# godk1122/IsaacLab

Measured on AMD Instinct MI355X. Metric: env-steps/sec (whole node), Anymal-C rough 4096 envs/GPU, RSL-RL PPO iteration (collect+GAE+update), higher is better.
Workload: dtype f32; 1 GPU; Isaac-Velocity-Rough-Anymal-C-v0, 4096 envs/GPU, T=24, 5 epochs x 4 minibatches, terrain 1204008 triangles, 4 state snapshots resident in HBM; parallelism=dp1, rollout=hipGraph, full_step=False, update=hipGraph (measured eager 16.00 ms, graph 15.55 ms), policy_params=571801

## Files before the change

include/imx.h:

```cpp
#ifndef IMX_H_
#define IMX_H_

#include <stddef.h>
#include <stdint.h>

#ifdef __cplusplus
extern "C" {
#endif

typedef struct imx_plan imx_plan_t;
typedef struct imx_mesh imx_mesh_t;
typedef void* imx_stream_t;

#define IMX_MAGIC 0x31584D49
#define IMX_PLAN_VERSION 3
#define IMX_HEADER_WORDS 48
#define IMX_MAX_OBS_GROUPS 4
#define IMX_REC_WORDS 20
#define IMX_FRAME_WORDS 9
#define IMX_FT_HEADER_WORDS 4

enum imx_header_word {
    IMX_H_MAGIC = 0, IMX_H_VERSION, IMX_H_J, IMX_H_B, IMX_H_H, IMX_H_A, IMX_H_D, IMX_H_R, IMX_H_NTERM, IMX_H_NREW,
    IMX_H_NOBS, IMX_H_NACT, IMX_H_MAX_EP_LEN, IMX_H_STEP_DT , IMX_H_TERM_OFF, IMX_H_REW_OFF, IMX_H_OBS_OFF,
// ... 408 lines not shown
size_t imx_gae_scratch_bytes(int64_t T, int64_t N);
int imx_gae(int64_t T, int64_t N, const float* rewards_d, const float* values_d, const uint8_t* dones_d,
            const float* last_values_d, float gamma, float lam, int normalize, float* returns_d,
            float* advantages_d, void* scratch_d, imx_stream_t stream);

size_t imx_ppo_scratch_bytes(int64_t M);
int imx_ppo_loss_fwd(int64_t M, int64_t A, const float* mu_d, const float* sigma_d, int64_t sigma_stride,
                     const float* actions_d, const float* old_logp_d, const float* old_mu_d, const float* old_sigma_d,
                     const float* advantages_d, const float* returns_d, const float* values_d, const float* old_values_d,
                     float clip_param, int use_clipped_value_loss, float value_loss_coef, float entropy_coef,
                     float* out8_d, float* accum5_d, void* scratch_d, imx_stream_t stream);
int imx_ppo_loss_bwd(int64_t M, int64_t A, const float* mu_d, const float* sigma_d, int64_t sigma_stride,
                     const float* actions_d, const float* old_logp_d, const float* advantages_d, const float* returns_d,
                     const float* values_d, const float* old_values_d, float clip_param, int use_clipped_value_loss,
                     float value_loss_coef, float entropy_coef, float grad_scale, float* dmu_d, float* dsigma_d,
                     float* dvalue_d, imx_stream_t stream);

size_t imx_colsum_scratch_bytes(void);
int imx_colsum(int64_t M, int64_t A, const float* x_d, const float* y_d, float* out_d, void* scratch_d, imx_stream_t stream);

int imx_adam_step(int64_t n, float* param_d, const float* grad_d, float* exp_avg_d, float* exp_avg_sq_d,
                  const float* lr_d, const float* grad_norm_d, float max_norm, float beta1, float beta2, float eps,
                  int64_t step, imx_stream_t stream);

int imx_adam_update(int64_t n, float* param_d, const float* grad_d, float* exp_avg_d, float* exp_avg_sq_d, float* state8_d,
                    const float* kl_d, float desired_kl, const float* grad_norm_d, float max_norm, float beta1,
                    float beta2, float eps, imx_stream_t stream);

size_t imx_adam_norm_scratch_bytes(int64_t n);
int imx_adam_update_norm(int64_t n, float* param_d, const float* grad_d, float* exp_avg_d, float* exp_avg_sq_d, float* state8_d,
                         const float* kl_d, float desired_kl, float max_norm, float beta1, float beta2, float eps,
                         void* scratch_d, size_t scratch_bytes, imx_stream_t stream);

int imx_gather_rows(int64_t M, const int64_t* idx_d, int n, const void* const* src_d, void* const* dst_d,
                    const int32_t* width_floats, imx_stream_t stream);
int imx_gather_rows_pitched(int64_t M, const int64_t* idx_d, int n, const void* const* src_d, void* const* dst_d,
                            const int32_t* width_floats, const int32_t* dst_pitch_floats, imx_stream_t stream);

int imx_policy_act(int64_t N, int64_t A, int64_t D, const float* mu_d, const float* std_d, const float* value_d,
                   const float* obs_d, uint64_t seed, const int32_t* step_counter_d, float* actions_out_d,
                   float* logp_out_d, float* mu_out_d, float* sigma_out_d, float* values_out_d, float* obs_out_d,
                   float* actions_env_d, imx_stream_t stream);

int imx_rollout_post(int64_t N, const float* reward_d, const uint8_t* terminated_d, const uint8_t* truncated_d,
                     const float* value_t_d, float gamma, int bootstrap_time_outs, float* rewards_out_d,
                     uint8_t* dones_out_d, int64_t* dones_long_d, float* cur_reward_sum_d, float* cur_ep_len_d,
                     float* ep_stats3_d, const float* log_in_d, float* log_accum_d, int num_log, imx_stream_t stream);


int imx_contact_sensor_update(int64_t N, int64_t B, int64_t H, const float* new_net_forces_d, float dt, float update_period,
                              float force_threshold, int track_air_time, float* timestamp_d,
                              float* timestamp_last_update_d, uint8_t* is_outdated_d, float* net_forces_w_d,
                              float* net_forces_w_history_d, float* last_air_time_d, float* current_air_time_d,
                              float* last_contact_time_d, float* current_contact_time_d, imx_stream_t stream);

int imx_velocity_command(int64_t N, const float* cfg15, int heading_command, float dt, int do_compute,
                         const float* root_quat_w_d,
                         const float* root_lin_vel_w_d, const float* root_ang_vel_w_d, const uint8_t* reset_mask_d,
                         const float* uniforms_d, uint64_t seed, const int32_t* step_counter_d, float* vel_command_b_d,
                         float* heading_target_d, uint8_t* is_heading_env_d, uint8_t* is_standing_env_d,
                         float* time_left_d, int64_t* command_counter_d, float* metric_error_vel_xy_d,
                         float* metric_error_vel_yaw_d, imx_stream_t stream);

int imx_pose_command(int64_t N, const float* cfg16, int make_quat_unique, int64_t body_idx, int64_t num_bodies, float dt,
                     int do_compute, const float* root_pos_w_d, const float* root_quat_w_d, const float* body_pos_w_d,
                     const float* body_quat_w_d, const uint8_t* reset_mask_d, const float* uniforms_d, uint64_t seed,
// ... 22 lines not shown
                          const float* weights_d, int64_t num_weights, const float* joint_pos_target_d, const float* joint_pos_d,
                          const float* joint_vel_d, float* hidden_state_d, float* cell_state_d, float saturation_effort,
                          const float* effort_limit_d, const float* velocity_limit_d, float* computed_effort_d,
                          float* applied_effort_d, imx_stream_t stream);

int imx_actuator_net_mlp(int64_t N, int64_t J, int num_dense, const int32_t* dense_out_h, int act, const float* weights_d,
                         int64_t num_weights, int history_length, const int32_t* input_idx_d, int num_idx, float pos_scale,
                         float vel_scale, float torque_scale, int vel_first, const float* joint_pos_target_d,
                         const float* joint_pos_d, const float* joint_vel_d, float* pos_error_history_d, float* vel_history_d,
                         float saturation_effort, const float* effort_limit_d, const float* velocity_limit_d,
                         float* computed_effort_d, float* applied_effort_d, imx_stream_t stream);

int imx_empirical_normalization(int64_t N, int64_t D, const float* x_d, int update, float eps, float* mean_d, float* var_d,
                                float* std_d, int64_t* count_d, float* out_d, imx_stream_t stream);

typedef struct imx_norm_group imx_norm_group_t;
typedef struct imx_infer_norm imx_infer_norm_t;
#include "imx_normalization_struct.h"
size_t imx_empirical_normalization_partials_bytes(int64_t N, int64_t D);
int imx_empirical_normalization_update(int ngroups, const imx_norm_group_t* groups, imx_stream_t stream);


size_t imx_mlp_scratch_bytes(int64_t M, int out_features, int in_features);

int imx_mlp_dw(int64_t M, int N, int K, const float* dY_d, int64_t ldy, const float* X_d, int64_t ldx, float* dW_d,
               float* db_d, void* scratch_d, size_t scratch_bytes, imx_stream_t stream);

typedef struct imx_reduce_batch imx_reduce_batch_t;
int imx_reduce_batch_create(imx_reduce_batch_t** out);
void imx_reduce_batch_destroy(imx_reduce_batch_t* batch);
int imx_mlp_set_dw_cu_budget(int cus);
int imx_reduce_batch_begin(imx_reduce_batch_t* batch);
int imx_reduce_batch_flush(imx_reduce_batch_t* batch, imx_stream_t stream);

int imx_mlp_dw_elu(int64_t M, int N, int K, const float* dH_d, int64_t ldg, const float* H_d, int64_t ldh, float elu_alpha,
                   float* dZ_out_d, int64_t ldd, const float* X_d, int64_t ldx, float* dW_d, float* db_d, void* scratch_d,
                   size_t scratch_bytes, imx_stream_t stream);

int imx_mlp_infer(int64_t M, const float* X_d, int64_t ldx, int nnets, const int* nlayers, const int* dims,
                  const float* const* weights_d, const int* weight_pitch, const float* const* biases_d, const float* elu_alpha,
                  float* const* out_d, imx_stream_t stream);

typedef struct imx_policy_act {
    const float* std_d;
    uint64_t seed;
    const int32_t* step_counter_d;
    float* actions_out_d;
    float* logp_out_d;
    float* mu_out_d;
    float* sigma_out_d;
    float* obs_out_d;
    const imx_plan_t* plan;
    const imx_state_t* state;
    const imx_buffers_t* buf;
    float pre_clip;
} imx_policy_act_t;
int imx_mlp_infer_act(int64_t M, const float* X_d, int64_t ldx, int nnets, const int* nlayers, const int* dims,
                      const float* const* weights_d, const int* weight_pitch, const float* const* packed_weights_d,
                      const float* const* biases_d, const float* elu_alpha, float* const* out_d, const imx_policy_act_t* act,
                      imx_stream_t stream);
int imx_mlp_infer_act2(int64_t M, const float* const* X_d, const int64_t* ldx, int nnets, const int* nlayers, const int* dims,
                       const float* const* weights_d, const int* weight_pitch, const float* const* packed_weights_d,
                       const float* const* biases_d, const float* elu_alpha, float* const* out_d, const imx_policy_act_t* act,
                       float* critic_obs_out_d, imx_stream_t stream);
int imx_mlp_infer_act2n(int64_t M, const float* const* X_d, const int64_t* ldx, int nnets, const int* nlayers, const int* dims,
                        const float* const* weights_d, const int* weight_pitch, const float* const* packed_weights_d,
// ... 112 lines not shown
```

isaaclab_amd/csrc/mlp.hip:

```cpp
#include <algorithm>

#include "imx_internal.h"
#include "imx_infer_device.h"


namespace {

constexpr int DW_T = 128;
constexpr int DW_BM = 32;
constexpr int DW_LD = DW_T + 32;

struct DwArgs {
    int64_t M;
    int N, K;
    const float* dY;
    int64_t ldy;
    const float* X;
    int64_t ldx;
    float* part;
    float* part_db;
    int tn, tk, S;
    int64_t rps;
    const float* H;
    int64_t ldh;
// ... 929 lines not shown
        else if (xvec) IMX_DW_LAUNCH(false, true, true);
        else IMX_DW_LAUNCH(false, false, true);
    } else {
        if (yvec && xvec) IMX_DW_LAUNCH(true, true, false);
        else if (yvec) IMX_DW_LAUNCH(true, false, false);
        else if (xvec) IMX_DW_LAUNCH(false, true, false);
        else IMX_DW_LAUNCH(false, false, false);
    }
#undef IMX_DW_LAUNCH
    IMX_HIP(hipGetLastError());
    return reduce_or_defer(who, (int64_t)N * K, p.S, a.part, dW_d, N, a.part_db, db_d, st);
}

extern "C" int imx_reduce_batch_create(imx_reduce_batch_t** out) {
    IMX_REQUIRE(out, "imx_reduce_batch_create: null argument");
    *out = new imx_reduce_batch();
    (*out)->args.n = 0;
    (*out)->blocks = 0;
    return 0;
}

extern "C" void imx_reduce_batch_destroy(imx_reduce_batch_t* b) {
    if (t_batch == b) t_batch = nullptr;
    delete b;
}

extern "C" int imx_reduce_batch_begin(imx_reduce_batch_t* b) {
    IMX_REQUIRE(b, "imx_reduce_batch_begin: null batch");
    IMX_REQUIRE(t_batch == nullptr, "imx_reduce_batch_begin: another batch is still open on this thread (flush it first)");
    t_batch = b;
    return 0;
}

extern "C" int imx_reduce_batch_flush(imx_reduce_batch_t* b, imx_stream_t stream) {
    IMX_REQUIRE(b && t_batch == b, "imx_reduce_batch_flush: this batch is not the one open on this thread");
    t_batch = nullptr;
    if (b->args.n == 0) return 0;
    hipLaunchKernelGGL(k_mlp_reduce_batch, dim3(b->blocks), dim3(64, RED_Y), 0, (hipStream_t)stream, b->args);
    b->args.n = 0;
    b->blocks = 0;
    IMX_HIP(hipGetLastError());
    return 0;
}

extern "C" int imx_mlp_dw(int64_t M, int N, int K, const float* dY_d, int64_t ldy, const float* X_d, int64_t ldx, float* dW_d,
                          float* db_d, void* scratch_d, size_t scratch_bytes, imx_stream_t stream) {
    return mlp_dw_launch("imx_mlp_dw", M, N, K, dY_d, ldy, nullptr, 0, 0.0f, nullptr, 0, X_d, ldx, dW_d, db_d, scratch_d, scratch_bytes,
                         stream);
}

extern "C" int imx_mlp_dw_elu(int64_t M, int N, int K, const float* dH_d, int64_t ldg, const float* H_d, int64_t ldh, float elu_alpha,
                              float* dZ_out_d, int64_t ldd, const float* X_d, int64_t ldx, float* dW_d, float* db_d, void* scratch_d,
                              size_t scratch_bytes, imx_stream_t stream) {
    IMX_REQUIRE(H_d, "imx_mlp_dw_elu: the saved activation output is required");
    return mlp_dw_launch("imx_mlp_dw_elu", M, N, K, dH_d, ldg, H_d, ldh, elu_alpha, dZ_out_d, ldd, X_d, ldx, dW_d, db_d, scratch_d,
                         scratch_bytes, stream);
}

static int head_fwd_launch(int64_t M, int K, int A, float* h_d, int64_t ldh, const float* W_d, const float* b_d, float* y_d,
                           int elu_in_place, float elu_alpha, const imx_head_loss_t* loss, imx_stream_t stream) {
    IMX_REQUIRE(M > 0 && h_d && W_d && b_d && y_d, "imx_mlp_head_fwd: bad arguments");
    IMX_REQUIRE(A >= 1 && A <= HEAD_A, "imx_mlp_head_fwd: %d outputs (1..%d supported; wider layers are library GEMMs)", A, HEAD_A);
    IMX_REQUIRE(K >= 16 && K % 16 == 0 && K <= 2048 && ldh >= K && ldh % 4 == 0 && aligned16(h_d),
                "imx_mlp_head_fwd: in-features %d (pitch %lld) must be a multiple of 16, 16-byte aligned rows", K, (long long)ldh);
    IMX_REQUIRE((size_t)A * K * sizeof(float) <= 64 * 1024, "imx_mlp_head_fwd: %d x %d weights do not fit the 64 KB of LDS used", A, K);
    imx_head_loss_t L{};
    int mode = 0;
    if (loss) {
        L = *loss;
        mode = L.mode;
        IMX_REQUIRE(mode == 1 || mode == 2, "imx_mlp_head_fwd_loss: mode %d (1 policy, 2 value)", mode);
        if (mode == 1) {
            IMX_REQUIRE(L.sigma_d && L.actions_d && L.old_logp_d && L.advantages_d && L.dmu_d && L.dsigma_d, "imx_mlp_head_fwd_loss: null policy argument");
            IMX_REQUIRE(L.sigma_stride == 0 || L.sigma_stride == A, "imx_mlp_head_fwd_loss: sigma_stride must be 0 (shared std) or A");
        } else {
// ... 519 lines not shown
```

isaaclab_amd/csrc/rollout.hip:

```cpp
#include "imx_internal.h"

struct Mom {
    float n, mean, m2;
};
IMX_DEV Mom mom_merge(Mom a, Mom b) {
    Mom r;
    r.n = a.n + b.n;
    if (r.n == 0.0f) { r.mean = 0.0f; r.m2 = 0.0f; return r; }
    const float d = b.mean - a.mean;
    r.mean = a.mean + d * (b.n / r.n);
    r.m2 = a.m2 + b.m2 + d * d * (a.n * b.n / r.n);
    return r;
}
IMX_DEV Mom mom_wave(Mom m) {
#pragma unroll
    for (int o = 32; o > 0; o >>= 1) {
        Mom b;
        b.n = __shfl_xor(m.n, o, 64);
        b.mean = __shfl_xor(m.mean, o, 64);
        b.m2 = __shfl_xor(m.m2, o, 64);
        const bool lo = ((threadIdx.x & o) == 0);
        m = lo ? mom_merge(m, b) : mom_merge(b, m);
    }
    return m;
// ... 456 lines not shown
}

extern "C" int imx_adam_update(int64_t n, float* p, const float* g, float* m, float* v, float* state8, const float* kl_d,
                               float desired_kl, const float* grad_norm_d, float max_norm, float beta1, float beta2,
                               float eps, imx_stream_t stream) {
    IMX_REQUIRE(n > 0 && p && g && m && v && state8, "imx_adam_update: bad arguments");
    hipLaunchKernelGGL(k_adam_prepare, dim3(1), dim3(64), 0, (hipStream_t)stream, state8, kl_d, desired_kl, grad_norm_d,
                       max_norm, beta1, beta2);
    const unsigned grid = (unsigned)std::min<int64_t>((n + 255) / 256, 2048);
    hipLaunchKernelGGL(k_adam_apply, dim3(grid), dim3(256), 0, (hipStream_t)stream, n, p, g, m, v, (const float*)state8, beta1,
                       beta2, eps);
    IMX_HIP(hipGetLastError());
    return 0;
}


static int adam_norm_blocks(int64_t n) {
    return (int)((n + (int64_t)ADAM_NORM_BLOCK * ADAM_NORM_PER_THREAD - 1) / ((int64_t)ADAM_NORM_BLOCK * ADAM_NORM_PER_THREAD));
}

extern "C" size_t imx_adam_norm_scratch_bytes(int64_t n) { return n > 0 ? ((size_t)adam_norm_blocks(n) + 1) * sizeof(float) : 0; }

extern "C" int imx_adam_update_norm(int64_t n, float* p, const float* g, float* m, float* v, float* state8, const float* kl_d,
                                    float desired_kl, float max_norm, float beta1, float beta2, float eps, void* scratch_d,
                                    size_t scratch_bytes, imx_stream_t stream) {
    IMX_REQUIRE(n > 0 && p && g && m && v && state8 && scratch_d, "imx_adam_update_norm: bad arguments");
    const int G = adam_norm_blocks(n);
    IMX_REQUIRE(scratch_bytes >= ((size_t)G + 1) * sizeof(float), "imx_adam_update_norm: scratch too small (see imx_adam_norm_scratch_bytes)");
    hipLaunchKernelGGL(k_adam_norm_prepare, dim3((unsigned)G), dim3(ADAM_NORM_BLOCK), 0, (hipStream_t)stream, n, g, state8, kl_d, desired_kl,
                       max_norm, beta1, beta2, (float*)scratch_d);
    const unsigned grid = (unsigned)std::min<int64_t>((n + 255) / 256, 2048);
    hipLaunchKernelGGL(k_adam_apply, dim3(grid), dim3(256), 0, (hipStream_t)stream, n, p, g, m, v, (const float*)state8, beta1,
                       beta2, eps);
    IMX_HIP(hipGetLastError());
    return 0;
}

struct GatherArgs {
    const float* src[12];
    float* dst[12];
    int width[12];
    int dpitch[12];
    int offset[13];
    int n;
};
__global__ void __launch_bounds__(256) k_gather_rows(int64_t M, const int64_t* __restrict__ idx, GatherArgs a) {
    const int lane = threadIdx.x & 63;
    const int64_t wave = ((int64_t)blockIdx.x * blockDim.x + threadIdx.x) >> 6, nw = ((int64_t)gridDim.x * blockDim.x) >> 6;
    for (int64_t r0 = 2 * wave; r0 < M; r0 += 2 * nw) {
        const int64_t r1 = r0 + 1;
        const bool two = r1 < M;
        const int64_t s0 = idx[r0], s1 = two ? idx[r1] : 0;
        for (int k = 0; k < a.n; ++k) {
            const int w = a.width[k], dp = a.dpitch[k];
            const float* __restrict__ src = a.src[k];
            float* __restrict__ dst = a.dst[k];
            for (int c = lane; c < w; c += 64) {
                const float v0 = src[s0 * w + c];
                const float v1 = two ? src[s1 * w + c] : 0.0f;
                dst[r0 * dp + c] = v0;
                if (two) dst[r1 * dp + c] = v1;
            }
        }
    }
}

// ... 158 lines not shown
```

isaaclab_amd/rsl_rl/ppo.py:

```python

from __future__ import annotations

import ctypes
import os

import torch
import torch.distributed as dist
import torch.nn as nn
import torch.nn.functional as F

from .. import _lib
from .._lib import check, lib
from .storage import RolloutStorage


class _FusedPPOLoss(torch.autograd.Function):
    @staticmethod
    def forward(ctx, mu, sigma, value, actions, old_logp, old_mu, old_sigma, adv, ret, old_value, clip, clipped, vcoef, ecoef):
        L = lib()
        M, A = mu.shape
        mu_c, sg_c, v_c = mu.contiguous(), sigma.contiguous(), value.contiguous()
        args = [t.contiguous() for t in (actions, old_logp, old_mu, old_sigma, adv, ret, old_value)]
        actions, old_logp, old_mu, old_sigma, adv, ret, old_value = args
        out8 = torch.empty(8, device=mu.device)
        scratch = torch.empty(int(L.imx_ppo_scratch_bytes(M)), dtype=torch.uint8, device=mu.device)
        check(L.imx_ppo_loss_fwd(M, A, mu_c.data_ptr(), sg_c.data_ptr(), A, actions.data_ptr(), old_logp.data_ptr(),
                                 old_mu.data_ptr(), old_sigma.data_ptr(), adv.data_ptr(), ret.data_ptr(), v_c.data_ptr(),
                                 old_value.data_ptr(), float(clip), int(clipped), float(vcoef), float(ecoef),
                                 out8.data_ptr(), None, scratch.data_ptr(), _lib.current_stream(mu.device)))
        ctx.save_for_backward(mu_c, sg_c, v_c, actions, old_logp, adv, ret, old_value)
        ctx.cfg = (float(clip), int(clipped), float(vcoef), float(ecoef))
        stats = out8[:4]
        ctx.mark_non_differentiable(stats)
        return out8[4], stats

    @staticmethod
    def backward(ctx, g_loss, _g_stats):
        mu, sigma, value, actions, old_logp, adv, ret, old_value = ctx.saved_tensors
        clip, clipped, vcoef, ecoef = ctx.cfg
        M, A = mu.shape
        dmu, dsigma, dvalue = torch.empty_like(mu), torch.empty_like(sigma), torch.empty_like(value)
        check(lib().imx_ppo_loss_bwd(M, A, mu.data_ptr(), sigma.data_ptr(), A, actions.data_ptr(), old_logp.data_ptr(),
                                     adv.data_ptr(), ret.data_ptr(), value.data_ptr(), old_value.data_ptr(), clip, clipped,
                                     vcoef, ecoef, 1.0, dmu.data_ptr(), dsigma.data_ptr(), dvalue.data_ptr(),
# ... 178 lines not shown

FUSED_L0 = os.getenv("IMX_FUSED_L0", "1") != "0"
FUSED_HEAD = os.getenv("IMX_FUSED_HEAD", "0")
LOSS_ON_SIDE = os.getenv("IMX_LOSS_ON_SIDE", "1") == "1"


def fused_first_layer_ok(x: torch.Tensor, w: torch.Tensor) -> bool:
    return (x.is_cuda and x.dtype == torch.float32 and x.stride(1) == 1 and w.is_contiguous() and w.shape[1] == x.shape[1]
            and x.shape[1] <= FUSED_FIRST_LAYER_MAX_K and FUSED_L0)


def mlp_scratch(layers, M: int, device) -> torch.Tensor:
    n = max(int(lib().imx_mlp_scratch_bytes(M, lin.out_features, lin.in_features)) for lin, _ in layers)
    return torch.empty(n, dtype=torch.uint8, device=device)


class DeferredReductions:

    def __init__(self, layers, M: int, device):
        import ctypes

        L = lib()
        self.scratch = [torch.empty(int(L.imx_mlp_scratch_bytes(M, lin.out_features, lin.in_features)), dtype=torch.uint8, device=device)
                        for lin, _ in layers]
        h = ctypes.c_void_p()
        check(L.imx_reduce_batch_create(ctypes.byref(h)))
        self.handle = h

    def __del__(self):
        try:
            lib().imx_reduce_batch_destroy(self.handle)
        except Exception:
            pass


def _head_bwd_args(scratch, which="a"):
    mode = FUSED_HEAD
    if mode == "0" or (mode == "c" and which != "c") or (mode == "a" and which != "a"):
        return None
    if isinstance(scratch, DeferredReductions):
        return {"scratch": scratch.scratch[-1], "batch": scratch.handle}
    return {"scratch": scratch, "batch": None}


def mlp_forward(layers, x, out=None, head_loss=None, first=None):
    saved = [x]
    h = x
    pending_elu = None
    for li, (lin, act) in enumerate(layers):
        if li == 0 and first is not None:
            h = first
            saved.append(h)
            continue
        if act is None and _is_head(lin, h):
            if out is not None and li == len(layers) - 1:
                z = out
            else:
                z = torch.empty(h.shape[0], lin.out_features, device=h.device, dtype=h.dtype)
            fb = head_loss.get("bwd") if head_loss is not None and li == len(layers) - 1 else None
            if (fb is not None and lin.in_features in (128, 256) and lin.out_features <= 16 and h.stride(0) % 4 == 0
                    and (pending_elu is not None or li == 0 or layers[li - 1][1] is None)):
                scr = fb["scratch"]
                dprev = torch.empty(h.shape[0], lin.in_features, device=h.device, dtype=h.dtype)
                check(lib().imx_mlp_head_fwd_bwd(h.shape[0], lin.in_features, lin.out_features, h.data_ptr(), h.stride(0), lin.weight.data_ptr(),
                                                 lin.bias.data_ptr(), z.data_ptr(), int(pending_elu is not None), float(pending_elu or 0.0),
                                                 ctypes.byref(head_loss["loss"]), dprev.data_ptr(), lin.weight.grad.data_ptr(),
# ... 15 lines not shown
        else:
            if pending_elu is not None:
                h = F.elu(h, alpha=pending_elu, inplace=True)
                pending_elu = None
            if li == 0 and isinstance(act, nn.ELU) and li + 1 < len(layers) - 1 and fused_first_layer_ok(h, lin.weight):
                z = torch.empty(h.shape[0], lin.out_features, device=h.device)
                check(lib().imx_mlp_fwd_elu(h.shape[0], lin.out_features, lin.in_features, h.data_ptr(), h.stride(0), lin.weight.data_ptr(),
                                            lin.bias.data_ptr(), float(act.alpha), 1, z.data_ptr(), z.stride(0), _lib.current_stream(h.device)))
                h = z
                saved.append(h)
                continue
            z = torch.addmm(lin.bias, h, lin.weight.t())
        if act is None:
            h = z
        elif isinstance(act, nn.ELU):
            nxt = layers[li + 1][0] if li + 1 < len(layers) else None
            if nxt is not None and layers[li + 1][1] is None and _is_head(nxt, z) and li + 1 == len(layers) - 1:
                pending_elu = float(act.alpha)
                h = z
            else:
                h = F.elu(z, alpha=act.alpha, inplace=True)
            saved.append(h)
        else:
            h = act(z)
            saved.append((z, h))
    if pending_elu is not None:
        h = F.elu(h, alpha=pending_elu, inplace=True)
    if out is not None and h is not out:
        out.copy_(h)
        h = out
    return h, saved


def mlp_backward(layers, saved, dout, scratch=None, head_dprev=None):
    L = lib()
    M = dout.shape[0]
    if scratch is None:
        scratch = mlp_scratch(layers, M, dout.device)
    stream = _lib.current_stream(dout.device)
    deferred = scratch if isinstance(scratch, DeferredReductions) else None
    if deferred is not None:
        check(L.imx_reduce_batch_begin(deferred.handle))
    try:
        _mlp_backward_layers(L, layers, saved, dout, M, scratch, deferred, stream, head_dprev)
    finally:
        if deferred is not None:
            check(L.imx_reduce_batch_flush(deferred.handle, stream))


def _mlp_backward_layers(L, layers, saved, dout, M, scratch, deferred, stream, head_dprev=None):
    d = dout
    pending = None
    top = len(layers) - 1
    if head_dprev is not None:
        d, top = head_dprev, top - 1
    for i in range(top, -1, -1):
        lin, _ = layers[i]
        x = saved[i] if not isinstance(saved[i], tuple) else saved[i][1]
        prev_act = layers[i - 1][1] if i > 0 else None
        N, K = lin.out_features, lin.in_features
        scr = deferred.scratch[i] if deferred is not None else scratch
        if pending is not None:
            dh, h, alpha = pending
            pending = None
            d = torch.empty_like(dh) if i > 0 else None
            check(L.imx_mlp_dw_elu(M, N, K, dh.data_ptr(), dh.stride(0), h.data_ptr(), h.stride(0), float(alpha),
                                   _lib.ptr(d), N, x.data_ptr(), x.stride(0), lin.weight.grad.data_ptr(),
                                   lin.bias.grad.data_ptr(), scr.data_ptr(), scr.numel(), stream))
        else:
            if not d.is_contiguous():
                d = d.contiguous()
            if i > 0 and _is_head(lin, x) and (prev_act is None or isinstance(prev_act, nn.ELU)):
                dprev = torch.empty(M, K, device=d.device, dtype=d.dtype)
                check(L.imx_mlp_head_bwd(M, K, N, d.data_ptr(), x.data_ptr(), x.stride(0), lin.weight.data_ptr(),
                                         float(prev_act.alpha) if prev_act is not None else 0.0, int(prev_act is not None),
                                         dprev.data_ptr(), lin.weight.grad.data_ptr(), lin.bias.grad.data_ptr(),
                                         scr.data_ptr(), scr.numel(), stream))
                d = dprev
                continue
            check(L.imx_mlp_dw(M, N, K, d.data_ptr(), d.stride(0), x.data_ptr(), x.stride(0), lin.weight.grad.data_ptr(),
                               lin.bias.grad.data_ptr(), scr.data_ptr(), scr.numel(), stream))
        if i > 0:
            dx = torch.mm(d, lin.weight)
            if isinstance(prev_act, nn.ELU) and dx.stride(1) == 1 and saved[i].stride(1) == 1:
                pending = (dx, saved[i], prev_act.alpha)
            elif isinstance(prev_act, nn.ELU):
                d = torch.ops.aten.elu_backward(dx, prev_act.alpha, 1.0, 1.0, True, saved[i])
            elif prev_act is None:
                d = dx
            else:
                z, h = saved[i]
                d = _act_backward(prev_act, dx, z, h)


def _act_backward(act, dh, z, h):
    if isinstance(act, nn.Identity):
        return dh
    if isinstance(act, nn.Tanh):
        return torch.ops.aten.tanh_backward(dh, h)
    if isinstance(act, nn.Sigmoid):
        return torch.ops.aten.sigmoid_backward(dh, h)
    if isinstance(act, nn.ReLU):
        return torch.ops.aten.threshold_backward(dh, h, 0)
    if isinstance(act, nn.LeakyReLU):
        return torch.ops.aten.leaky_relu_backward(dh, z, act.negative_slope, False)
    if isinstance(act, nn.SELU):
        return torch.ops.aten.elu_backward(dh, 1.6732632423543772848170429916717, 1.0507009873554804934193349852946, 1.0, False, z)
    with torch.inference_mode(False), torch.enable_grad():
        zz = z.clone().requires_grad_(True)
        (d,) = torch.autograd.grad(act(zz), zz, dh.clone())
    return d


class PPO:
# ... 5 lines not shown
        if kwargs:
            raise NotImplementedError("PPO got arguments it does not implement: " + ", ".join(sorted(kwargs)))
        if rnd_cfg is not None or symmetry_cfg is not None:
            raise NotImplementedError("RND / symmetry augmentation are outside the hot-path scope (SURVEY.md section 8)")
        self.device = torch.device(device)
        self.is_multi_gpu = multi_gpu_cfg is not None
        if self.is_multi_gpu:
            self.gpu_global_rank = multi_gpu_cfg["global_rank"]
            self.gpu_world_size = multi_gpu_cfg["world_size"]
        else:
            self.gpu_global_rank, self.gpu_world_size = 0, 1
        self.policy = policy.to(self.device)
        pair = self._first_layer_pair()
        self.bucket = FlatParams(self.policy, extra_slots=8,
                                 first=() if pair is None else (pair[0].weight, pair[1].weight, pair[0].bias, pair[1].bias))
        self._joint0 = None
        if pair is not None:
            la, lc, _alpha = pair
            H, K = la.out_features, la.in_features
            if (lc.weight.data_ptr() == la.weight.data_ptr() + 4 * H * K and lc.bias.data_ptr() == la.bias.data_ptr() + 4 * H
                    and la.weight.is_contiguous() and lc.weight.is_contiguous()):
                w0 = self.bucket.flat[:2 * H * K].view(2 * H, K)
                b0 = self.bucket.flat[2 * H * K:2 * H * K + 2 * H]
                if w0.data_ptr() == la.weight.data_ptr() and b0.data_ptr() == la.bias.data_ptr():
                    self._joint0 = (w0, b0, H, float(pair[2]))
        self.storage: RolloutStorage | None = None
        self.transition = RolloutStorage.Transition()
        self.clip_param, self.num_learning_epochs, self.num_mini_batches = clip_param, num_learning_epochs, num_mini_batches
        self.value_loss_coef, self.entropy_coef, self.gamma, self.lam = value_loss_coef, entropy_coef, gamma, lam
        self.max_grad_norm, self.use_clipped_value_loss = max_grad_norm, use_clipped_value_loss
        self.desired_kl, self.schedule = desired_kl, schedule
        self.normalize_advantage_per_mini_batch = normalize_advantage_per_mini_batch
        self.betas, self.eps = (0.9, 0.999), 1e-8
        self._adam = torch.tensor([float(learning_rate), 0.0, 1.0, 1.0, 1.0, 0.0, 1.0, 0.0], device=self.device)
        self._stats = torch.zeros(5, device=self.device)
        self._out8 = self.bucket.grad[self.bucket.numel:self.bucket.numel + 8]
        self._kl = self._out8[3:4]
        self._norm_scratch = torch.zeros(int(lib().imx_adam_norm_scratch_bytes(self.bucket.numel)), dtype=torch.uint8, device=self.device) \
            if self.device.type == "cuda" else None
        self._actor_layers = _mlp_layers(self.policy.actor)
        self._critic_layers = _mlp_layers(self.policy.critic)
        self._ws: dict = {}
        self._side = None
        if self.device.type == "cuda" and os.getenv("IMX_DW_CU_BUDGET"):
            lib().imx_mlp_set_dw_cu_budget(int(os.environ["IMX_DW_CU_BUDGET"]))
        self.two_streams = bool(two_streams)
        if self.device.type == "cuda":
            for st in (self._side_stream(), self._aux_stream()):
                if st is not None:
                    with torch.cuda.stream(st):
                        torch.zeros(1, device=self.device)
            torch.cuda.synchronize(self.device)

    @property
    def learning_rate(self) -> float:
        return float(self._adam[0].item())

    def optimizer_state_dict(self) -> dict:
        base = self.bucket.flat.data_ptr()
        state, params = {}, []
        step = self._adam[1:2].clone().reshape(())
        for i, p in enumerate(q for q in self.policy.parameters() if q.requires_grad):
            off = (p.data_ptr() - base) // 4
            params.append(i)
            if float(step) > 0:
                state[i] = {"step": step.clone(), "exp_avg": self.bucket.exp_avg[off:off + p.numel()].view_as(p).clone(),
                            "exp_avg_sq": self.bucket.exp_avg_sq[off:off + p.numel()].view_as(p).clone()}
# ... 100 lines not shown
    time_allreduce = False
    _allreduce_events: list = []

    def reduce_parameters(self):
        if self.time_allreduce and self.device.type == "cuda":
            e0, e1 = torch.cuda.Event(enable_timing=True), torch.cuda.Event(enable_timing=True)
            e0.record()
            allreduce_mean_(self.bucket.grad, self.gpu_world_size)
            e1.record()
            self._allreduce_events.append((e0, e1))
            return
        allreduce_mean_(self.bucket.grad, self.gpu_world_size)

    def allreduce_us(self) -> dict | None:
        ev, self._allreduce_events = self._allreduce_events, []
        if not ev:
            return None
        ev[-1][1].synchronize()
        t = [a.elapsed_time(b) * 1e3 for a, b in ev]
        return {"mean": sum(t) / len(t), "max": max(t), "count": len(t)}

    def _side_stream(self):
        if not self.two_streams or self.device.type != "cuda":
            return None
        if self._side is None:
            self._side = torch.cuda.Stream(self.device)
        return self._side

    def _aux_stream(self):
        if getattr(self, "_aux", None) is None:
            self._aux = torch.cuda.Stream(self.device)
        return self._aux

    def _workspace(self, M: int, A: int):
        ws = self._ws.get((M, A))
        if ws is None:
            dev = self.device
            ws = dict(dmu=torch.empty(M, A, device=dev), dsigma=torch.empty(M, A, device=dev), dvalue=torch.empty(M, 1, device=dev),
                      scratch=torch.empty(int(lib().imx_ppo_scratch_bytes(M)), dtype=torch.uint8, device=dev),
                      colsum=torch.empty(int(lib().imx_colsum_scratch_bytes()), dtype=torch.uint8, device=dev),
                      mlp_a=DeferredReductions(self._actor_layers, M, dev), mlp_c=DeferredReductions(self._critic_layers, M, dev))
            self._ws[(M, A)] = ws
        return ws

    def minibatch_step(self, obs, critic_obs, actions, target_values, advantages, returns, old_logp, old_mu, old_sigma):
        L = lib()
        pol = self.policy
        stream = _lib.current_stream(self.device)
        M, A = actions.shape
        for name, t in (("actions", actions), ("target_values", target_values), ("advantages", advantages), ("returns", returns),
                        ("old_actions_log_prob", old_logp), ("old_mu", old_mu), ("old_sigma", old_sigma)):
            if not t.is_contiguous():
                raise _lib.ImxError(f"PPO.minibatch_step: {name} must be contiguous (shape {tuple(t.shape)}, strides {t.stride()})")
        ws = self._workspace(M, A)
        if pol.noise_std_type == "scalar":
            sigma, sstride = pol.std, 0
        else:
            sigma, sstride = None, A
        clipf, vclip = float(self.clip_param), int(self.use_clipped_value_loss)
        vcoef, ecoef = float(self.value_loss_coef), float(self.entropy_coef)

        heads = {"a": None, "c": None}

        def actor_pass(st):
            nonlocal sigma
            hl = None
# ... 24 lines not shown
            if not hl.get("applied"):
                check(L.imx_ppo_loss_bwd(M, A, None, None, sstride, None, None, None, returns.data_ptr(), value.data_ptr(),
                                         target_values.data_ptr(), clipf, vclip, vcoef, ecoef, 1.0, None, None, ws["dvalue"].data_ptr(), st))
            return value, saved_c

        def loss_values(mu, value, st):
            check(L.imx_ppo_loss_fwd(M, A, mu.data_ptr(), sigma.data_ptr(), sstride, actions.data_ptr(), old_logp.data_ptr(),
                                     old_mu.data_ptr(), old_sigma.data_ptr(), advantages.data_ptr(), returns.data_ptr(),
                                     value.data_ptr(), target_values.data_ptr(), clipf, vclip, vcoef, ecoef,
                                     self._out8.data_ptr(), self._stats.data_ptr(), ws["scratch"].data_ptr(), st))
            if pol.noise_std_type == "scalar" and A <= 64:
                check(L.imx_colsum(M, A, ws["dsigma"].data_ptr(), None, pol.std.grad.data_ptr(), ws["colsum"].data_ptr(), st))
            elif A <= 64:
                check(L.imx_colsum(M, A, ws["dsigma"].data_ptr(), sigma.data_ptr(), pol.log_std.grad.data_ptr(), ws["colsum"].data_ptr(), st))
            elif pol.noise_std_type == "scalar":
                torch.sum(ws["dsigma"], dim=0, out=pol.std.grad)
            else:
                torch.sum(ws["dsigma"] * sigma, dim=0, out=pol.log_std.grad)

        first_a = first_c = z0 = None
        joint_elu = None
        if self._joint0 is not None and critic_obs.data_ptr() == obs.data_ptr() and critic_obs.shape == obs.shape:
            w0, b0, H0, alpha0 = self._joint0
            if fused_first_layer_ok(obs, w0):
                z0 = torch.empty(obs.shape[0], 2 * H0, device=obs.device)
                check(L.imx_mlp_fwd_elu(obs.shape[0], 2 * H0, obs.shape[1], obs.data_ptr(), obs.stride(0), w0.data_ptr(), b0.data_ptr(),
                                        alpha0, 1, z0.data_ptr(), z0.stride(0), stream))
            else:
                z0 = torch.addmm(b0, obs, w0.t())
                joint_elu = alpha0
            first_a, first_c = z0[:, :H0], z0[:, H0:]
        side = self._side_stream()
        main = torch.cuda.current_stream(self.device)
        if side is not None:
            loss_on_side = LOSS_ON_SIDE
            aux = self._aux_stream()
            side.wait_stream(main)
            if joint_elu is not None:
                F.elu(first_a, alpha=joint_elu, inplace=True)
            mu, saved_a = actor_pass(stream)
            mu_ready = torch.cuda.Event()
            mu_ready.record(main)
            with torch.cuda.stream(side):
                if joint_elu is not None:
                    F.elu(first_c, alpha=joint_elu, inplace=True)
                value, saved_c = critic_pass(side.cuda_stream)
                value_ready = torch.cuda.Event()
                value_ready.record(side)
            if not loss_on_side:
                aux.wait_stream(main)
                aux.wait_event(value_ready)
            mlp_backward(self._actor_layers, saved_a, ws["dmu"], ws["mlp_a"], head_dprev=heads["a"])
            with torch.cuda.stream(side):
                mlp_backward(self._critic_layers, saved_c, ws["dvalue"], ws["mlp_c"], head_dprev=heads["c"])
                if loss_on_side:
                    side.wait_event(mu_ready)
                    loss_values(mu, value, side.cuda_stream)
            if not loss_on_side:
                with torch.cuda.stream(aux):
                    loss_values(mu, value, aux.cuda_stream)
            main.wait_stream(side)
            if not loss_on_side:
                main.wait_stream(aux)
            mu.record_stream(aux)
            mu.record_stream(side)
            value.record_stream(aux)
            value.record_stream(main)
            if z0 is not None:
                z0.record_stream(side)
        else:
            if joint_elu is not None:
                F.elu(z0, alpha=joint_elu, inplace=True)
            mu, saved_a = actor_pass(stream)
            value, saved_c = critic_pass(stream)
            loss_values(mu, value, stream)
            mlp_backward(self._actor_layers, saved_a, ws["dmu"], ws["mlp_a"], head_dprev=heads["a"])
            mlp_backward(self._critic_layers, saved_c, ws["dvalue"], ws["mlp_c"], head_dprev=heads["c"])
        return self._out8

    update_graph = False
    _update_calls = 0
    _update_g = None
    _update_t = None

    @torch.no_grad()
    def update(self):
        if not (self.update_graph and self.device.type == "cuda" and not self.is_multi_gpu) or self._update_t == "eager":
            return self._update_eager()
        self._update_calls += 1
        c = self._update_calls
        if c == 1:
            return self._update_eager()
        if c == 2:
            ev = [torch.cuda.Event(enable_timing=True) for _ in range(4)]
            self._update_ev = ev
            ev[0].record()
            out = self._update_eager()
            ev[1].record()
            return out
        if c == 5 and self._update_t is None and os.getenv("IMX_UPDATE_GRAPH") == "force":
            self._update_t = "graph"
        if c == 5 and self._update_t is None:
            ev = self._update_ev
            ev[3].synchronize()
            t_eager, t_graph = ev[0].elapsed_time(ev[1]), ev[2].elapsed_time(ev[3])
            self._update_times_ms = (t_eager, t_graph)
            self._update_t = "graph" if t_graph < t_eager else "eager"
            if self._update_t == "eager":
                self._update_g = None
                return self._update_eager()
# ... 7 lines not shown
            if c == 4:
                self._update_ev[2].record()
            self._update_g.replay()
            if c == 4:
                self._update_ev[3].record()
        self.storage.clear()
        return self._stats

    def _update_eager(self):
        b = self.bucket
        L = lib()
        stream = _lib.current_stream(self.device)
        self._stats.zero_()
        adaptive = self.desired_kl is not None and self.schedule == "adaptive"
        side = self._side_stream()
        copy_stream = self._aux_stream() if side is not None else None
        main = torch.cuda.current_stream(self.device) if side is not None else None
        gen = iter(self.storage.mini_batch_generator(self.num_mini_batches, self.num_learning_epochs, copy_stream=copy_stream))
        item = next(gen, None)
        while item is not None:
            if copy_stream is not None:
                batch, ready = item
                main.wait_event(ready)
            else:
                batch = item
            if self.normalize_advantage_per_mini_batch:
                batch = list(batch)
                adv = batch[4]
                batch[4] = (adv - adv.mean()) / (adv.std() + 1e-8)
            self.minibatch_step(*batch)
            item = next(gen, None)
            if self.is_multi_gpu:
                self.reduce_parameters()
            check(L.imx_adam_update_norm(b.numel, b.flat.data_ptr(), b.grad.data_ptr(), b.exp_avg.data_ptr(), b.exp_avg_sq.data_ptr(),
                                         self._adam.data_ptr(), self._kl.data_ptr() if adaptive else None,
                                         float(self.desired_kl or 0.0), float(self.max_grad_norm or 0.0), self.betas[0],
                                         self.betas[1], self.eps, self._norm_scratch.data_ptr(), self._norm_scratch.numel(), stream))
        if copy_stream is not None:
            main.wait_stream(copy_stream)
        self.storage.clear()
        return self._stats

    def loss_dict(self) -> dict:
        s = self._stats.tolist()
        n = max(s[4], 1.0)
        return {"value_function": s[0] / n, "surrogate": s[1] / n, "entropy": s[2] / n, "kl": s[3] / n}
```

Baseline: 5.484 million env-steps/s.

## Compute Adam grad-norm partials early during backward and split update kernel

Splits the fused Adam norm+update into a block-partial squared-norm kernel and an apply kernel. The partial sums for actor parameter blocks above the input layer are computed during the backward pass, once their gradients are final, so only the remaining late blocks are reduced before the update. The Adam state is double-banked so the apply kernel can read the old state and write a new one without a separate finalize kernel. This shortens the serial tail after backward, but adds launches, a 4096-thread-block tree reduction, and host-side bank bookkeeping that must stay consistent with graph capture.

Result: no change. 5.481 million env-steps/s (-0.0%).

```diff
diff --git a/include/imx.h b/include/imx.h
--- a/include/imx.h
+++ b/include/imx.h
@@ -464,6 +464,13 @@
                          const float* kl_d, float desired_kl, float max_norm, float beta1, float beta2, float eps,
                          void* scratch_d, size_t scratch_bytes, imx_stream_t stream);
 
+#define IMX_ADAM_NORM_BLOCK 4096
+int imx_adam_norm_partials(int64_t n, const float* grad_d, const int32_t* blocks_d, int count, void* scratch_d, size_t scratch_bytes,
+                           imx_stream_t stream);
+int imx_adam_update_partials(int64_t n, float* param_d, const float* grad_d, float* exp_avg_d, float* exp_avg_sq_d,
+                             const float* state8_in_d, float* state8_out_d, const float* kl_d, float desired_kl, float max_norm,
+                             float beta1, float beta2, float eps, const void* scratch_d, size_t scratch_bytes, imx_stream_t stream);
+
 int imx_gather_rows(int64_t M, const int64_t* idx_d, int n, const void* const* src_d, void* const* dst_d,
                     const int32_t* width_floats, imx_stream_t stream);
 int imx_gather_rows_pitched(int64_t M, const int64_t* idx_d, int n, const void* const* src_d, void* const* dst_d,
@@ -552,6 +559,7 @@
 int imx_mlp_set_dw_cu_budget(int cus);
 int imx_reduce_batch_begin(imx_reduce_batch_t* batch);
 int imx_reduce_batch_flush(imx_reduce_batch_t* batch, imx_stream_t stream);
+int imx_reduce_batch_flush_queued(imx_reduce_batch_t* batch, imx_stream_t stream);
 
 int imx_mlp_dw_elu(int64_t M, int N, int K, const float* dH_d, int64_t ldg, const float* H_d, int64_t ldh, float elu_alpha,
                    float* dZ_out_d, int64_t ldd, const float* X_d, int64_t ldx, float* dW_d, float* db_d, void* scratch_d,
diff --git a/isaaclab_amd/csrc/mlp.hip b/isaaclab_amd/csrc/mlp.hip
--- a/isaaclab_amd/csrc/mlp.hip
+++ b/isaaclab_amd/csrc/mlp.hip
@@ -985,15 +985,24 @@
     return 0;
 }
 
-extern "C" int imx_reduce_batch_flush(imx_reduce_batch_t* b, imx_stream_t stream) {
-    IMX_REQUIRE(b && t_batch == b, "imx_reduce_batch_flush: this batch is not the one open on this thread");
-    t_batch = nullptr;
+static int reduce_batch_launch(imx_reduce_batch* b, imx_stream_t stream) {
     if (b->args.n == 0) return 0;
     hipLaunchKernelGGL(k_mlp_reduce_batch, dim3(b->blocks), dim3(64, RED_Y), 0, (hipStream_t)stream, b->args);
     b->args.n = 0;
     b->blocks = 0;
     IMX_HIP(hipGetLastError());
     return 0;
+}
+
+extern "C" int imx_reduce_batch_flush(imx_reduce_batch_t* b, imx_stream_t stream) {
+    IMX_REQUIRE(b && t_batch == b, "imx_reduce_batch_flush: this batch is not the one open on this thread");
+    t_batch = nullptr;
+    return reduce_batch_launch(b, stream);
+}
+
+extern "C" int imx_reduce_batch_flush_queued(imx_reduce_batch_t* b, imx_stream_t stream) {
+    IMX_REQUIRE(b && t_batch == b, "imx_reduce_batch_flush_queued: this batch is not the one open on this thread");
+    return reduce_batch_launch(b, stream);
 }
 
 extern "C" int imx_mlp_dw(int64_t M, int N, int K, const float* dY_d, int64_t ldy, const float* X_d, int64_t ldx, float* dW_d,
diff --git a/isaaclab_amd/csrc/rollout.hip b/isaaclab_amd/csrc/rollout.hip
--- a/isaaclab_amd/csrc/rollout.hip
+++ b/isaaclab_amd/csrc/rollout.hip
@@ -512,6 +512,104 @@
     const unsigned grid = (unsigned)std::min<int64_t>((n + 255) / 256, 2048);
     hipLaunchKernelGGL(k_adam_apply, dim3(grid), dim3(256), 0, (hipStream_t)stream, n, p, g, m, v, (const float*)state8, beta1,
                        beta2, eps);
+    IMX_HIP(hipGetLastError());
+    return 0;
+}
+
+static_assert(ADAM_NORM_BLOCK * ADAM_NORM_PER_THREAD == IMX_ADAM_NORM_BLOCK, "imx.h: IMX_ADAM_NORM_BLOCK");
+
+IMX_DEV float adam_norm_tree(float* red, float s) {
+    red[threadIdx.x] = s;
+    __syncthreads();
+    for (int w = ADAM_NORM_BLOCK / 2; w > 0; w >>= 1) {
+        if ((int)threadIdx.x < w) red[threadIdx.x] += red[threadIdx.x + w];
+        __syncthreads();
+    }
+    return red[0];
+}
+
+__global__ void __launch_bounds__(ADAM_NORM_BLOCK)
+k_adam_norm_partials(int64_t n, const float* __restrict__ g, const int32_t* __restrict__ blocks, int G, float* __restrict__ scratch) {
+    __shared__ float red[ADAM_NORM_BLOCK];
+    const int b = blocks[blockIdx.x];
+    if (b < 0 || b >= G) return;
+    const int64_t base = (int64_t)b * ADAM_NORM_BLOCK * ADAM_NORM_PER_THREAD;
+    float s = 0.0f;
+#pragma unroll
+    for (int k = 0; k < ADAM_NORM_PER_THREAD; ++k) {
+        const int64_t i = base + (int64_t)k * ADAM_NORM_BLOCK + threadIdx.x;
+        if (i < n) s += g[i] * g[i];
+    }
+    const float tot = adam_norm_tree(red, s);
+    if (threadIdx.x == 0) scratch[b] = tot;
+}
+
+__global__ void __launch_bounds__(ADAM_NORM_BLOCK)
+k_adam_apply_partials(int64_t n, float* __restrict__ p, const float* __restrict__ g, float* __restrict__ m, float* __restrict__ v,
+                      const float* __restrict__ st, float* __restrict__ st_out, const float* __restrict__ kl_d, float desired_kl,
+                      float max_norm, float b1, float b2, float eps, const float* __restrict__ scratch, int G) {
+    __shared__ float red[ADAM_NORM_BLOCK];
+    const int64_t stride = (int64_t)gridDim.x * blockDim.x;
+    int64_t i = (int64_t)blockIdx.x * blockDim.x + threadIdx.x;
+    float g0 = 0.0f, m0 = 0.0f, v0 = 0.0f, p0 = 0.0f;
+    if (i < n) { g0 = g[i]; m0 = m[i]; v0 = v[i]; p0 = p[i]; }
+    float part = 0.0f;
+    for (int b = threadIdx.x; b < G; b += ADAM_NORM_BLOCK) part += scratch[b];
+    const float norm = sqrtf(adam_norm_tree(red, part));
+    float lr = st[0];
+    if (kl_d) {
+        const float kl = kl_d[0];
+        if (kl > desired_kl * 2.0f) lr = fmaxf(1.0e-5f, lr / 1.5f);
+        else if (kl < desired_kl / 2.0f && kl > 0.0f) lr = fminf(1.0e-2f, lr * 1.5f);
+    }
+    const float p1 = st[2] * b1, p2 = st[3] * b2;
+    const float coef = max_norm > 0.0f ? fminf(max_norm / (norm + 1.0e-6f), 1.0f) : 1.0f;
+    const float step_size = lr / (1.0f - p1), sqrt_bias2 = sqrtf(1.0f - p2);
+    if (blockIdx.x == 0 && threadIdx.x == 0) {
+        st_out[0] = lr;
+        st_out[1] = st[1] + 1.0f;
+        st_out[2] = p1;
+        st_out[3] = p2;
+        st_out[4] = coef;
+        st_out[5] = step_size;
+        st_out[6] = sqrt_bias2;
+        st_out[7] = norm;
+    }
+    for (bool first = true; i < n; i += stride, first = false) {
+        if (!first) { g0 = g[i]; m0 = m[i]; v0 = v[i]; p0 = p[i]; }
+        const float gi = g0 * coef;
+        const float mi = b1 * m0 + (1.0f - b1) * gi;
+        const float vi = b2 * v0 + (1.0f - b2) * gi * gi;
+        m[i] = mi;
+        v[i] = vi;
+        p[i] = p0 - step_size * (mi / (sqrtf(vi) / sqrt_bias2 + eps));
+    }
+}
+
+extern "C" int imx_adam_norm_partials(int64_t n, const float* g, const int32_t* blocks_d, int count, void* scratch_d, size_t scratch_bytes,
+                                      imx_stream_t stream) {
+    IMX_REQUIRE(n > 0 && g && count >= 0 && (blocks_d || count == 0) && scratch_d, "imx_adam_norm_partials: bad arguments");
+    const int G = adam_norm_blocks(n);
+    IMX_REQUIRE(count <= G, "imx_adam_norm_partials: %d blocks listed, the bucket has %d", count, G);
+    IMX_REQUIRE(scratch_bytes >= ((size_t)G + 1) * sizeof(float), "imx_adam_norm_partials: scratch too small (see imx_adam_norm_scratch_bytes)");
+    if (count == 0) return 0;
+    hipLaunchKernelGGL(k_adam_norm_partials, dim3((unsigned)count), dim3(ADAM_NORM_BLOCK), 0, (hipStream_t)stream, n, g, blocks_d, G,
+                       (float*)scratch_d);
+    IMX_HIP(hipGetLastError());
+    return 0;
+}
+
+extern "C" int imx_adam_update_partials(int64_t n, float* p, const float* g, float* m, float* v, const float* state8_in, float* state8_out,
+                                        const float* kl_d, float desired_kl, float max_norm, float beta1, float beta2, float eps,
+                                        const void* scratch_d, size_t scratch_bytes, imx_stream_t stream) {
+    IMX_REQUIRE(n > 0 && p && g && m && v && state8_in && state8_out && scratch_d, "imx_adam_update_partials: bad arguments");
+    IMX_REQUIRE(state8_in + 8 <= state8_out || state8_out + 8 <= state8_in,
+                "imx_adam_update_partials: the old and the new state must be different buffers (two banks, alternating)");
+    const int G = adam_norm_blocks(n);
+    IMX_REQUIRE(scratch_bytes >= ((size_t)G + 1) * sizeof(float), "imx_adam_update_partials: scratch too small (see imx_adam_norm_scratch_bytes)");
+    const unsigned grid = (unsigned)std::min<int64_t>((n + ADAM_NORM_BLOCK - 1) / ADAM_NORM_BLOCK, 2048);
+    hipLaunchKernelGGL(k_adam_apply_partials, dim3(grid), dim3(ADAM_NORM_BLOCK), 0, (hipStream_t)stream, n, p, g, m, v, state8_in,
+                       state8_out, kl_d, desired_kl, max_norm, beta1, beta2, eps, (const float*)scratch_d, G);
     IMX_HIP(hipGetLastError());
     return 0;
 }
diff --git a/isaaclab_amd/rsl_rl/ppo.py b/isaaclab_amd/rsl_rl/ppo.py
--- a/isaaclab_amd/rsl_rl/ppo.py
+++ b/isaaclab_amd/rsl_rl/ppo.py
@@ -9,7 +9,7 @@
 import torch.nn as nn
 import torch.nn.functional as F
 
-from .. import _lib
+from .. import _abi, _lib
 from .._lib import check, lib
 from .storage import RolloutStorage
 
@@ -254,6 +254,25 @@
             lib().imx_reduce_batch_destroy(self.handle)
         except Exception:
             pass
+
+
+NORM_BLOCK = _abi.DEFINES["IMX_ADAM_NORM_BLOCK"]
+
+
+def norm_block_sets(numel: int, early: dict) -> dict:
+    G = -(-numel // NORM_BLOCK)
+    covered, owner = [0] * G, [None] * G
+    for tag, ranges in early.items():
+        for off, n in ranges:
+            for b in range(off // NORM_BLOCK, -(-(off + n) // NORM_BLOCK) if n > 0 else 0):
+                covered[b] += min(off + n, (b + 1) * NORM_BLOCK) - max(off, b * NORM_BLOCK)
+                owner[b] = tag if owner[b] in (None, tag) else "late"
+    out = {tag: [] for tag in early}
+    out["late"] = []
+    for b in range(G):
+        full = covered[b] == min(numel, (b + 1) * NORM_BLOCK) - b * NORM_BLOCK
+        out[owner[b] if full and owner[b] is not None else "late"].append(b)
+    return out
 
 
 def _head_bwd_args(scratch, which="a"):
@@ -335,7 +354,7 @@
     return h, saved
 
 
-def mlp_backward(layers, saved, dout, scratch=None, head_dprev=None):
+def mlp_backward(layers, saved, dout, scratch=None, head_dprev=None, early=None):
     L = lib()
     M = dout.shape[0]
     if scratch is None:
@@ -344,20 +363,26 @@
     deferred = scratch if isinstance(scratch, DeferredReductions) else None
     if deferred is not None:
         check(L.imx_reduce_batch_begin(deferred.handle))
+        if early is not None:
+            where, fn = early
+            early = (where, lambda: fn(lambda st: check(L.imx_reduce_batch_flush_queued(deferred.handle, st))))
     try:
-        _mlp_backward_layers(L, layers, saved, dout, M, scratch, deferred, stream, head_dprev)
+        _mlp_backward_layers(L, layers, saved, dout, M, scratch, deferred, stream, head_dprev, early if deferred is not None else None)
     finally:
         if deferred is not None:
             check(L.imx_reduce_batch_flush(deferred.handle, stream))
 
 
-def _mlp_backward_layers(L, layers, saved, dout, M, scratch, deferred, stream, head_dprev=None):
+def _mlp_backward_layers(L, layers, saved, dout, M, scratch, deferred, stream, head_dprev=None, early=None):
     d = dout
     pending = None
     top = len(layers) - 1
     if head_dprev is not None:
         d, top = head_dprev, top - 1
     for i in range(top, -1, -1):
+        if early is not None and i == 0:
+            early[1]()
+            early = None
         lin, _ = layers[i]
         x = saved[i] if not isinstance(saved[i], tuple) else saved[i][1]
         prev_act = layers[i - 1][1] if i > 0 else None
@@ -383,6 +408,9 @@
                 continue
             check(L.imx_mlp_dw(M, N, K, d.data_ptr(), d.stride(0), x.data_ptr(), x.stride(0), lin.weight.grad.data_ptr(),
                                lin.bias.grad.data_ptr(), scr.data_ptr(), scr.numel(), stream))
+        if early is not None and i == 1 and early[0] == "dw":
+            early[1]()
+            early = None
         if i > 0:
             dx = torch.mm(d, lin.weight)
             if isinstance(prev_act, nn.ELU) and dx.stride(1) == 1 and saved[i].stride(1) == 1:
@@ -454,7 +482,8 @@
         self.desired_kl, self.schedule = desired_kl, schedule
         self.normalize_advantage_per_mini_batch = normalize_advantage_per_mini_batch
         self.betas, self.eps = (0.9, 0.999), 1e-8
-        self._adam = torch.tensor([float(learning_rate), 0.0, 1.0, 1.0, 1.0, 0.0, 1.0, 0.0], device=self.device)
+        self._adam_banks = torch.tensor([[float(learning_rate), 0.0, 1.0, 1.0, 1.0, 0.0, 1.0, 0.0], [0.0] * 8], device=self.device)
+        self._adam, self._adam_bank = self._adam_banks[0], 0
         self._stats = torch.zeros(5, device=self.device)
         self._out8 = self.bucket.grad[self.bucket.numel:self.bucket.numel + 8]
         self._kl = self._out8[3:4]
@@ -621,6 +650,52 @@
             self._aux = torch.cuda.Stream(self.device)
         return self._aux
 
+    early_tail_on_branch = False
+    early_tail_nets = ("a",)
+    _tail = None
+
+    def _split_tail(self):
+        if self.is_multi_gpu or self.device.type != "cuda":
+            return None
+        if self._tail is None:
+            base, numel = self.bucket.flat.data_ptr(), self.bucket.numel
+
+            def above_input(layers):
+                ps = [p for lin, _ in layers[1:] for p in (lin.weight, lin.bias) if p is not None and p.requires_grad]
+                return [((p.data_ptr() - base) // 4, p.numel()) for p in ps if 0 <= p.data_ptr() - base < 4 * numel]
+
+            early = {"a": above_input(self._actor_layers), "c": above_input(self._critic_layers)}
+            sets = norm_block_sets(numel, {k: v if k in self.early_tail_nets else [] for k, v in early.items()})
+            self._tail = {k: torch.tensor(v, dtype=torch.int32, device=self.device) for k, v in sets.items()}
+        return self._tail
+
+    def _norm_partials(self, blocks, stream):
+        b = self.bucket
+        check(lib().imx_adam_norm_partials(b.numel, b.grad.data_ptr(), blocks.data_ptr(), blocks.numel(), self._norm_scratch.data_ptr(),
+                                           self._norm_scratch.numel(), stream))
+
+    def _early_tail(self, tag, joins):
+        tail = self._split_tail()
+        if tail is None or tag not in self.early_tail_nets:
+            return None
+
+        def fn(flush):
+            if not self.early_tail_on_branch:
+                st = _lib.current_stream(self.device)
+                flush(st)
+                self._norm_partials(tail[tag], st)
+                return
+            aux = self._aux_stream()
+            aux.wait_stream(torch.cuda.current_stream(self.device))
+            with torch.cuda.stream(aux):
+                flush(aux.cuda_stream)
+                self._norm_partials(tail[tag], aux.cuda_stream)
+                done = torch.cuda.Event()
+                done.record(aux)
+            joins.append(done)
+
+        return ("dw" if self.early_tail_on_branch else "dx", fn)
+
     def _workspace(self, M: int, A: int):
         ws = self._ws.get((M, A))
         if ws is None:
@@ -711,6 +786,7 @@
             first_a, first_c = z0[:, :H0], z0[:, H0:]
         side = self._side_stream()
         main = torch.cuda.current_stream(self.device)
+        joins = []
         if side is not None:
             loss_on_side = LOSS_ON_SIDE
             aux = self._aux_stream()
@@ -729,9 +805,9 @@
             if not loss_on_side:
                 aux.wait_stream(main)
                 aux.wait_event(value_ready)
-            mlp_backward(self._actor_layers, saved_a, ws["dmu"], ws["mlp_a"], head_dprev=heads["a"])
+            mlp_backward(self._actor_layers, saved_a, ws["dmu"], ws["mlp_a"], head_dprev=heads["a"], early=self._early_tail("a", joins))
             with torch.cuda.stream(side):
-                mlp_backward(self._critic_layers, saved_c, ws["dvalue"], ws["mlp_c"], head_dprev=heads["c"])
+                mlp_backward(self._critic_layers, saved_c, ws["dvalue"], ws["mlp_c"], head_dprev=heads["c"], early=self._early_tail("c", joins))
                 if loss_on_side:
                     side.wait_event(mu_ready)
                     loss_values(mu, value, side.cuda_stream)
@@ -753,8 +829,10 @@
             mu, saved_a = actor_pass(stream)
             value, saved_c = critic_pass(stream)
             loss_values(mu, value, stream)
-            mlp_backward(self._actor_layers, saved_a, ws["dmu"], ws["mlp_a"], head_dprev=heads["a"])
-            mlp_backward(self._critic_layers, saved_c, ws["dvalue"], ws["mlp_c"], head_dprev=heads["c"])
+            mlp_backward(self._actor_layers, saved_a, ws["dmu"], ws["mlp_a"], head_dprev=heads["a"], early=self._early_tail("a", joins))
+            mlp_backward(self._critic_layers, saved_c, ws["dvalue"], ws["mlp_c"], head_dprev=heads["c"], early=self._early_tail("c", joins))
+        for done in joins:
+            main.wait_event(done)
         return self._out8
 
     update_graph = False
@@ -828,10 +906,22 @@
             item = next(gen, None)
             if self.is_multi_gpu:
                 self.reduce_parameters()
-            check(L.imx_adam_update_norm(b.numel, b.flat.data_ptr(), b.grad.data_ptr(), b.exp_avg.data_ptr(), b.exp_avg_sq.data_ptr(),
-                                         self._adam.data_ptr(), self._kl.data_ptr() if adaptive else None,
-                                         float(self.desired_kl or 0.0), float(self.max_grad_norm or 0.0), self.betas[0],
-                                         self.betas[1], self.eps, self._norm_scratch.data_ptr(), self._norm_scratch.numel(), stream))
+            kl_ptr = self._kl.data_ptr() if adaptive else None
+            tail = self._split_tail()
+            if tail is None:
+                check(L.imx_adam_update_norm(b.numel, b.flat.data_ptr(), b.grad.data_ptr(), b.exp_avg.data_ptr(), b.exp_avg_sq.data_ptr(),
+                                             self._adam.data_ptr(), kl_ptr, float(self.desired_kl or 0.0), float(self.max_grad_norm or 0.0), self.betas[0],
+                                             self.betas[1], self.eps, self._norm_scratch.data_ptr(), self._norm_scratch.numel(), stream))
+                continue
+            self._norm_partials(tail["late"], stream)
+            check(L.imx_adam_update_partials(b.numel, b.flat.data_ptr(), b.grad.data_ptr(), b.exp_avg.data_ptr(), b.exp_avg_sq.data_ptr(),
+                                             self._adam_banks[self._adam_bank].data_ptr(), self._adam_banks[1 - self._adam_bank].data_ptr(),
+                                             kl_ptr, float(self.desired_kl or 0.0), float(self.max_grad_norm or 0.0), self.betas[0],
+                                             self.betas[1], self.eps, self._norm_scratch.data_ptr(), self._norm_scratch.numel(), stream))
+            self._adam_bank ^= 1
+        if self._adam_bank:
+            self._adam_banks[0].copy_(self._adam_banks[1])
+            self._adam_bank = 0
         if copy_stream is not None:
             main.wait_stream(copy_stream)
         self.storage.clear()
```
